# Gadersd/stable-diffusion-xl-burn

Hardware: AMD Instinct MI355X
Metric: images/sec SDXL-base 1024x1024 30-step CFG7.5 (whole job); UNet step ms p50 (higher is better)
Workload: dtype f16; 1 GPU; SDXL-base 1024x1024, n_steps=30 (31 CFG UNet step pairs), CFG 7.5, batch 1 prompt/GPU + VAE decode to u8 (BASELINE configs[1]); precision=f16, vae_dtype=f32_split, weights=synthetic seeded (random-init SDXL-base architecture), mix_classes=0, parallelism=replica x1, 1 prompt per GPU, weights broadcast once over RCCL, hipgraph=True, split_cfg=False, fused_xattn=True, pipelined_decode=False, prompts_per_call=1, full=False, library=stable-diffusion-xl-burn_amd/lib/libsdxl_mi355.so, debug_set=

## Files before the change

### stable-diffusion-xl-burn_amd/csrc/capi.hip

```cpp
#include "capi_internal.h"
#include <algorithm>
#include <cstring>

using namespace sdxl;

thread_local std::string sdxl::g_err;

namespace {
template <class H, class F> void create_handle(sdxl_ctx* ctx, H** out, F make) {
  std::unique_ptr<H> h(new H());
  h->ctx = ctx;
  make(*h);
  *out = h.release();
}
UNetCfg to_cfg(const sdxl_unet_config* c) {
  SDXL_REQUIRE(c != nullptr, "null config");
  SDXL_REQUIRE(c->n_levels >= 1 && c->n_levels <= 8, "n_levels out of range");
  UNetCfg u;
  u.adm_in_channels = c->adm_in_channels; u.in_channels = c->in_channels; u.out_channels = c->out_channels;
  u.model_channels = c->model_channels; u.n_head_channels = c->n_head_channels; u.context_dim = c->context_dim;
  u.is_refiner = c->is_refiner != 0;
  for (int i = 0; i < c->n_levels; ++i) { u.channel_mults.push_back(c->channel_mults[i]); u.transformer_depths.push_back(c->transformer_depths[i]); }
  SDXL_REQUIRE(u.model_channels > 0 && u.n_head_channels > 0 && u.context_dim > 0 && u.adm_in_channels > 0, "bad UNet config");
  return u;
// ... 72 lines not shown
  c->device = device_id;
  SDXL_HIP(hipStreamCreate(&c->stream));
  igemm_glds_init();
  attention_init();
  *out = c;
  API_END
}
int sdxl_debug_set(const char* key, int value) {
  API_BEGIN
  SDXL_REQUIRE(key != nullptr, "null key");
  if (std::strcmp(key, "igemm_variant") == 0) igemm_set_variant(value);
  else if (std::strcmp(key, "attn_variant") == 0) attention_set_variant(value);
  else if (std::strcmp(key, "igemm_epilogue_staged") == 0) igemm_set_epilogue_staged(value);
  else if (std::strcmp(key, "hl_weights_exact") == 0) igemm_set_hl_weights_exact(value);
  else if (std::strcmp(key, "igemm_wreg") == 0) igemm_set_wreg(value);
  else if (std::strcmp(key, "igemm_tsw") == 0) igemm_set_tsw(value);
  else if (std::strcmp(key, "igemm_warm") == 0) igemm_set_warm(value);
  else if (std::strcmp(key, "attn_xsplit") == 0) attention_set_xsplit(value);
  else if (std::strcmp(key, "splitk_wt") == 0) igemm_set_splitk_wt(value);
  else if (std::strcmp(key, "hl_demote") == 0) unet_set_hl_demote(value);
  else if (std::strcmp(key, "mix_classes") == 0) unet_set_mix_classes(value);
  else if (std::strcmp(key, "hl_tile96") == 0) igemm_set_hl_tile96(value);
  else if (std::strcmp(key, "wreg_xcd2d") == 0) igemm_set_wreg_xcd2d(value);
  else if (std::strcmp(key, "wide_db") == 0) igemm_set_wide_db(value);
#ifdef SDXL_MEASURE
  else if (std::strcmp(key, "igemm_unrolled") == 0) igemm_set_unrolled(value);
  else if (std::strcmp(key, "xa_vec64") == 0) igemm_set_xa_vec64(value);
  else if (std::strcmp(key, "no_cfg") == 0) g_debug_no_cfg = value != 0;
#endif
  else throw Error(std::string("unknown debug key ") + key);
// ... 539 lines not shown
```

### stable-diffusion-xl-burn_amd/csrc/capi_ops.hip

```cpp
#include "capi_internal.h"
#include <algorithm>
#include <cmath>

using namespace sdxl;

namespace {
__global__ void transpose_pad_kernel(const float* src, int lds_, int rows, int C, void* dst, int dt, int ldd) {
  const size_t i = (size_t)blockIdx.x * blockDim.x + threadIdx.x;
  if (i >= (size_t)rows * C) return;
  const int r = i / C, c = i - (size_t)r * C;
  const float v = src[(size_t)r * lds_ + c];
  if (dt == DT_F16) reinterpret_cast<_Float16*>(dst)[(size_t)c * ldd + r] = (_Float16)v;
  else reinterpret_cast<float*>(dst)[(size_t)c * ldd + r] = v;
}
__global__ void causal_mask_kernel(float* out, int n) {
  const int i = blockIdx.x * blockDim.x + threadIdx.x;
  if (i >= n * n) return;
  const int r = i / n, c = i - r * n;
  out[i] = c > r ? -INFINITY : 0.f;
}

struct Operand { std::string name; std::vector<int> shape; int kind; const float* data = nullptr; float eps = 0.f; int ld = 0; };
using Operands = std::vector<Operand>;
void add_linear(Operands& o, const std::string& n, int K, int N, const float* w, const float* b, int ld = 0) {
// ... 385 lines not shown
                                  const float* wq, const float* k, const float* v, int B, int Nq, int Nk, int C, int fused,
                                  float* out) {
  API_BEGIN
  SDXL_REQUIRE(ctx && x && gamma && beta && wq && k && v && out, "null argument");
  SDXL_REQUIRE(C % 64 == 0 && B >= 1 && Nq >= 1 && Nk >= 1, "State size must be a multiple of head size");
  use(ctx);
  hipStream_t s = pick(ctx, stream);
  const int M = B * Nq, vt_ld = (int)round_up(Nk, 64), H = C / 64;
  SDXL_REQUIRE(!fused || igemm_xattn_ok(DT_F16, DT_F16, M, C, C, Nq, Nk), "fused cross-attention: unsupported shape");
  Operands ops;
  add_linear(ops, "lin", C, C, wq, nullptr);
  add_norm(ops, "norm", C, gamma, beta, eps);
  Packed pk(ops, DT_F16, s);
  Tmp tmp;
  Exec ex; ex.s = s; ex.cdt = DT_F16; ex.sdt = DT_F16;
  const Lin l = pk.wb.linear_ln("lin", false, "norm");
  const F16Stream xs = identity_producer(ex, tmp, x, M, C, s);
  const Act xi(xs.rows, C, DT_F16);
  void* od = tmp.get((size_t)M * C * 2);
  Epi e; e.ln_stat = xs.stat; e.rpb = Nq;
  if (fused == 3) {
    float* q32 = (float*)tmp.get((size_t)M * C * 4);
    run_linear(ex, l, xi, M, Act(q32, C, DT_F32), e);
    void* khl = tmp.get((size_t)B * Nk * C * 4);
    void* vhl = tmp.get((size_t)B * C * vt_ld * 4);
    launch_f32_to_hl(k, C, khl, C, (size_t)B * Nk, C, s);
    launch_f32_to_hl(stage_vt(tmp, v, B, Nk, C, DT_F32, vt_ld, s), vt_ld, vhl, vt_ld, (size_t)B * C, vt_ld, s);
    AttnParams p = attn_params(q32, khl, vhl, vt_ld, od, C, DT_HL, B, H, Nq, Nk);
    p.q_dt = DT_F32; p.o_dt = DT_F16;
    SDXL_REQUIRE(launch_attention_d64_hl(p, s), "split-operand attention: unsupported shape");
  } else if (fused == 2) {
// ... 157 lines not shown
```

### stable-diffusion-xl-burn_amd/csrc/engine.h

```cpp
#pragma once
#include "kernels.h"

#include <map>
#include <memory>
#include <stdexcept>
#include <string>
#include <utility>
#include <vector>

namespace sdxl {

struct Error : std::runtime_error {
  explicit Error(const std::string& m) : std::runtime_error(m) {}
};
#define SDXL_HIP(x)                                                                                   \
  do {                                                                                                \
    hipError_t e__ = (x);                                                                             \
    if (e__ != hipSuccess) throw ::sdxl::Error(std::string(#x) + " failed: " + hipGetErrorString(e__)); \
  } while (0)
#define SDXL_REQUIRE(cond, msg)                          \
  do {                                                   \
    if (!(cond)) throw ::sdxl::Error(std::string(msg));  \
  } while (0)

// ... 96 lines not shown
  int dt;
  hipStream_t st;
  float* tmp = nullptr; size_t tmp_numel = 0;
  std::string last_fetched;
  WeightBuilder(const std::vector<ParamSpec>& sp, WeightSource& s, DeviceArena& a, int dtype, hipStream_t stream);
  ~WeightBuilder();
  bool wfrag = true;
  static size_t arena_bound(const std::vector<ParamSpec>& specs, int dt, bool wfrag = true);
  const ParamSpec& spec(const std::string& name, size_t* idx = nullptr) const;
  bool has(const std::string& name) const { return index.count(name) != 0; }
  const float* fetch(const std::string& name);
  Lin linear(const std::string& name, bool geglu = false, int dt_override = -1);
  Lin fused_linear(const std::vector<std::string>& names, int dt_override = -1);
  Lin linear_hilo(const std::string& name, bool geglu, bool dup = false, bool hl_interleave = false);
  float hl_scale(Lin& l, const std::vector<std::string>& weight_names);
  Lin linear_ln(const std::string& name, bool geglu, const std::string& norm);
  Lin fused_linear_ln(const std::vector<std::string>& names, const std::string& norm);
  Lin fold_ln(const std::vector<std::string>& names, const std::string& norm, bool geglu, int dt_override = -1, bool shadow = false, Lin* plain = nullptr, bool hilo_dup = false,
              bool hl_interleave = false);
  bool all_f16_exact(const std::vector<std::string>& names);
  float* tmp2 = nullptr; size_t tmp2_numel = 0;
  Lin conv(const std::string& name);
  void attach_wfrag(Lin& l, bool fill);
  NormW norm(const std::string& name);
};

struct Act {
  void* p = nullptr; int ld = 0; int dt = DT_F16;
  const float* gn_part = nullptr; int gn_rt = 0;
  const float* a_scale = nullptr;
  int a_scale_n = 1;
  Act() {}
  Act(void* p_, int ld_, int dt_) : p(p_), ld(ld_), dt(dt_) {}
  Act cols(int c0) const { Act a((char*)p + (size_t)c0 * dt_size(dt), ld, dt); a.a_scale = a_scale; a.a_scale_n = a_scale_n; return a; }
};

struct Profiler {
  enum { IGEMM = 0, ATTENTION = 1, GROUPNORM = 2, LAYERNORM = 3, OTHER = 4, NCLS = 5 };
// ... 322 lines not shown
```

### stable-diffusion-xl-burn_amd/csrc/igemm_common.h

```cpp
#pragma once
#include "kernels.h"
#include <stdexcept>
#include <type_traits>

namespace sdxl {

typedef _Float16 half_t;
typedef _Float16 half8 __attribute__((ext_vector_type(8)));
typedef _Float16 half4 __attribute__((ext_vector_type(4)));
typedef float f32x4 __attribute__((ext_vector_type(4)));
typedef float f32x16 __attribute__((ext_vector_type(16)));

typedef const __attribute__((address_space(1))) void* gptr_t;
typedef float f32x8 __attribute__((ext_vector_type(8)));
__device__ __forceinline__ f32x8 uniform_load8(const float* ptr) {
  const unsigned long long a = (unsigned long long)(uintptr_t)ptr;
  const unsigned long long u = ((unsigned long long)__builtin_amdgcn_readfirstlane((unsigned)(a >> 32)) << 32) | (unsigned)__builtin_amdgcn_readfirstlane((unsigned)a);
  return *(const __attribute__((address_space(4))) f32x8*)(uintptr_t)u;
}
__device__ __forceinline__ f32x4 col_vec4(const float* arr, bool present, int nbu, int fh, const void* zeros) {
  const f32x8 c = uniform_load8(present ? arr + nbu : reinterpret_cast<const float*>(zeros));
  return fh ? f32x4{c[4], c[5], c[6], c[7]} : f32x4{c[0], c[1], c[2], c[3]};
}
typedef __attribute__((address_space(3))) void* lptr_t;
// ... 888 lines not shown
    const float inv = 1.0f / l;
#pragma unroll
    for (int dt = 0; dt < 2; ++dt) {
      f32x16 o;
#pragma unroll
      for (int r = 0; r < 16; ++r) o[r] = 0.f;
#pragma unroll
      for (int s6 = 0; s6 < 6; ++s6) o = __builtin_amdgcn_mfma_f32_32x32x16_f16(vf[dt][s6], pf[s6], o, 0, 0, 0);
#pragma unroll
      for (int r = 0; r < 16; ++r) acc[i][dt][r] = o[r] * inv;
    }
    lnA[i] = 1.f; lnC[i] = 0.f;
  }
}

template <int TM>
__device__ __forceinline__ void xattn_inplace_hl(const IgemmParams& p, f32x16 (&acc)[TM][2], int mw, int nw, int lane,
                                                 float (&lnA)[TM], float (&lnC)[TM], const void* zeros) {
  static_assert(TM == 1, "split-precision fused cross-attention: one-MFMA-row wave tiles");
  if (nw >= p.N) return;
  const int fh = lane >> 5;
  const int nctx = p.xa_nctx;
  const int mclamp = mw < p.M ? mw : p.M - 1;
  const int b = __builtin_amdgcn_readfirstlane(mclamp / p.rpb);
  const size_t foff = ((size_t)b * (p.N >> 6) + (nw >> 6)) * (24 * 64) + lane;
  const half8* fhi = reinterpret_cast<const half8*>(p.xa_k) + foff;
  const half8* flo = reinterpret_cast<const half8*>(p.xa_k_lo) + foff;
  half8 kh[3][4], kl[3][4];
#pragma unroll
  for (int t = 0; t < 3; ++t)
// ... 94 lines not shown
```

### stable-diffusion-xl-burn_amd/csrc/igemm_glds.hip

```cpp
#include "igemm_common.h"
#include <atomic>

namespace sdxl {

template <int BM, int BN, int NS, int MINB = 2>
__global__ __launch_bounds__(256, MINB) void igemm_glds_kernel(const IgemmParams p, const void* zeros) {
  kernarg_prefetch<(int)sizeof(IgemmParams) + 8>();
  constexpr int WM = BM / 2, WN = BN / 2;
  constexpr int TM = WM / 32, TN = WN / 32;
  constexpr int AJ = BM / 32, BJ = BN / 32;
  constexpr int PER = AJ + BJ;
  constexpr int KT = 64;
  constexpr int STAGE = (BM + BN) * 128;
  extern __shared__ __attribute__((aligned(16))) char smem[];

  const int tid = threadIdx.x, lane = tid & 63;
  const int wave = __builtin_amdgcn_readfirstlane(tid >> 6);
  const int wm = wave >> 1, wn = wave & 1;

  const int tilesN = (p.N + BN - 1) / BN;
  const int nwg = gridDim.x;
  int bid = blockIdx.x;
  {
    const int q = nwg >> 3, r = nwg & 7, xcd = bid & 7, idx = bid >> 3;
// ... 994 lines not shown
      const int g = f - 12, d = 32 * (g / 6) + fr, key = 16 * (g % 6) + sub;
      if (key < nctx) x = Vt[((size_t)b * C + h * 64 + d) * vt_ld + key];
    }
    v[e] = x;
  }
  out[i] = v;
}
size_t xattn_pack_bytes(int B, int C) { return (size_t)B * (C / 64) * 24 * 64 * 16; }
void launch_xattn_pack(const void* K, const void* Vt, void* out, int B, int C, int nctx, int vt_ld, hipStream_t s) {
  const size_t n = (size_t)B * (C / 64) * 24 * 64;
  hipLaunchKernelGGL(xattn_pack_kernel, dim3((unsigned)((n + 255) / 256)), dim3(256), 0, s, reinterpret_cast<const half_t*>(K),
                     reinterpret_cast<const half_t*>(Vt), reinterpret_cast<half8*>(out), B, C, nctx, vt_ld);
}

bool launch_igemm_wreg(const IgemmParams& p, int variant, hipStream_t s);
bool launch_igemm_glds(const IgemmParams& p, int variant, hipStream_t s) {
  if (!g_zero_pages[current_device()]) return false;
  if (p.act > 1) return false;
  if (p.a_dt != DT_F16 || (p.Cin % 64) != 0 || (p.lda % 8) != 0 || (p.Kpad % 64) != 0) return false;
  if ((reinterpret_cast<uintptr_t>(p.A) & 15) != 0) return false;
  if (p.n_split < p.N && (p.n_split & 3) != 0) return false;
  if (p.ebias && (p.ebias_ld & 3) != 0) return false;
  if (p.stat_out && (variant == 2 || variant == 5 || variant == 19 || variant == 38)) return false;
  const bool was_auto = variant == 0;
  IgemmParams psk = p;
  psk.splitk = 1;
  psk.splitk_wt = g_splitk_wt.load();
  if (p.xa_k) {
    if (p.act != 0 || p.n_split < p.N || p.stat_out || p.R || p.ebias ||
        !igemm_xattn_ok(p.a_dt, p.c_dt, p.M, p.N, p.K, p.rpb, p.xa_nctx))
      throw std::runtime_error("igemm: fused cross-attention needs a plain f16 projection (no residual / split outputs)");
    if (!p.xa_k_lo && p.c_dt != DT_F16) throw std::runtime_error("igemm: the f16 fused cross-attention writes f16 rows");
    const int nk = p.Kpad / 64;
    if (p.xa_k_lo) {
      const double c128 = tile_cost(p.M, p.N, nk, 128, 128, 1.0), c96 = tile_cost(p.M, p.N, nk, 96, 128, 1.0);
      if (c96 < c128) launch_pipe<96, 128, 3, 3, 6, half_t, true, false, false, true>(psk, s);
      else launch_pipe<128, 128, 4, 4, 8, half_t, true, false, false, true>(psk, s);
      return true;
    }
    int v = variant;
    if (v != 35 && v != 36 && v != 44 && v != 45) {
      const double c256 = tile_cost(p.M, p.N, nk, 256, 128, 1.0), c128 = tile_cost(p.M, p.N, nk, 128, 128, 1.0), c96 = tile_cost(p.M, p.N, nk, 96, 128, 1.0);
      v = c256 <= c128 && c256 <= c96 ? 35 : (c96 < c128 ? 45 : (nk >= 40 ? 44 : 36));
    }
    if (v == 35) launch_pipe<256, 128, 3, 4, 8, half_t, true>(psk, s);
    else if (v == 36) launch_pipe<128, 128, 4, 4, 8, half_t, true>(psk, s);
    else if (v == 44) launch_pipe<128, 128, 5, 4, 8, half_t, true>(psk, s);
    else launch_pipe<96, 128, 3, 3, 6, half_t, true>(psk, s);
    return true;
  }
  if (p.gn_part) {
    if (!igemm_gn_part_ok(p)) throw std::runtime_error("igemm: GroupNorm statistics requested from a shape the 256x128 epilogue does not take");
    variant = 0;
  }
  if (p.shadow) {
// ... 116 lines not shown
```

### stable-diffusion-xl-burn_amd/csrc/igemm_wreg.hip

```cpp
#include "igemm_common.h"
#include <atomic>

namespace sdxl {

template <int OFF> __device__ __forceinline__ half8 wreg_gload128(const half_t* ptr) {
  half8 v;
  asm volatile("global_load_dwordx4 %0, %1, off offset:%2" : "=v"(v) : "v"(ptr), "n"(OFF));
  return v;
}

__global__ void repack_wfrag_kernel(const f32x4* __restrict__ src, f32x4* __restrict__ dst, int nblocks, int nk) {
  const size_t i = (size_t)blockIdx.x * blockDim.x + threadIdx.x;
  const size_t total = (size_t)nblocks * nk * 256;
  if (i >= total) return;
  const int lane = (int)(i & 63), kk = (int)((i >> 6) & 3);
  const size_t t = i >> 8;
  const int kt = (int)(t % nk);
  const int nb = (int)(t / nk);
  dst[i] = src[(size_t)(nb * 32 + (lane & 31)) * (nk * 8) + kt * 8 + kk * 2 + (lane >> 5)];
}
void launch_repack_wfrag(const void* w, void* wf, int Npad, int Kpad, hipStream_t s) {
  const int nblocks = Npad / 32, nk = Kpad / 64;
  const size_t total = (size_t)nblocks * nk * 256;
  hipLaunchKernelGGL(repack_wfrag_kernel, dim3((unsigned)((total + 255) / 256)), dim3(256), 0, s, reinterpret_cast<const f32x4*>(w),
// ... 137 lines not shown
  if (part == 0 && fh == 0) {
#pragma unroll
    for (int i = 0; i < TM; ++i) {
      const int r2 = (i * 32 + fr) * 2;
      const float s1 = (A1[i] + xsum[r2]) + (xsum[TM * 64 + r2] + xsum[2 * TM * 64 + r2]);
      const float s2 = (A2[i] + xsum[r2 + 1]) + (xsum[TM * 64 + r2 + 1] + xsum[2 * TM * 64 + r2 + 1]);
      if (mok[i]) {
        float* dst = p.stat_out + ((size_t)(nw >> 6) * p.M + m[i]) * 2;
        dst[0] = piv[i] + s1 * (1.0f / 64.0f);
        dst[1] = fmaxf(s2 - s1 * s1 * (1.0f / 64.0f), 0.f);
      }
    }
  }
}

#ifdef SDXL_MEASURE
__device__ unsigned* g_wreg_tl = nullptr;
void igemm_set_wreg_timeline(void* buf) {
  unsigned* b = reinterpret_cast<unsigned*>(buf);
  if (hipMemcpyToSymbol(HIP_SYMBOL(g_wreg_tl), &b, sizeof(b)) != hipSuccess) throw std::runtime_error("igemm_wreg: cannot set the timeline buffer");
}
#define WREG_STAMP(i) do { wtl[i] = (unsigned)__builtin_amdgcn_s_memtime(); } while (0)
#else
#define WREG_STAMP(i) do { } while (0)
#endif
constexpr int wreg_mode_flags(int m) {
  return m >= 16 ? m : m == 1 ? 16 : m == 2 ? 32 : m == 3 ? 64 : m == 4 ? 128 : m == 5 ? 256 : m == 6 ? 512 : m == 7 ? 1024 : m == 8 ? 2048 : 0;
}
template <int BM, int L, int MODE = 0>
__global__ __launch_bounds__(512) void igemm_wreg_kernel(const IgemmParams p, const void* zeros) {
#ifdef SDXL_MEASURE
  unsigned wtl[8] = {0, 0, 0, 0, 0, 0, 0, 0};
  wtl[6] = (unsigned)__builtin_amdgcn_s_memrealtime();
#endif
  WREG_STAMP(0);
  kernarg_prefetch<(int)sizeof(IgemmParams) + 8>();
  constexpr int NG = 2;
  constexpr int NSG = L + 1;
  constexpr int TM = BM / 32;
  constexpr int PP = BM / 32;
  constexpr int FL = wreg_mode_flags(MODE);
  constexpr bool NOMFMA = FL & 16, FROZEN = FL & 32, NOVMEM = FL & 64, NOBAR = FL & 128, XCDALT = FL & 256, NOA = FL & 512, NOWL = FL & 1024,
                 ACONTIG = FL & 2048, NOLDS = FL & 4096;
  constexpr int NW = NOWL ? 0 : 4;
// ... 184 lines not shown
    for (int pass = (ns - first) / NSG; pass > 0; --pass) {
      static_for<L>([&](auto C) { ktile(std::integral_constant<int, decltype(C)::value + 1>{}, STEADY{}); });
      ktile(I0{}, STEADY{});
    }
  }
  static_for<L>([&](auto X) {
    constexpr int D = L - decltype(X)::value;
    if (D <= nkg) ktile(std::integral_constant<int, L + 1 - D>{}, std::integral_constant<int, D>{});
  });
  WREG_STAMP(3);
  if constexpr (!NOBAR) { if ((nk & 1) && g == 1) __builtin_amdgcn_s_barrier(); }
  asm volatile("" ::: "memory");
  __builtin_amdgcn_sched_barrier(0);

  WregEpiOperands<TM> eop;
  wreg_epilogue_request<TM>(p, m0, n0 + w * 32, lane, g, zeros, eop);
  static_assert(4 * TM * 2 * 64 * 16 <= L * SLOT, "a group's four exchange pieces must fit its dead slots 0 .. L - 1");
  f32x4* xw = reinterpret_cast<f32x4*>(smem + g * RING) + (size_t)w * (TM * 2 * 64) + lane;
  const f32x4* xo = reinterpret_cast<const f32x4*>(smem + (1 - g) * RING) + (size_t)w * (TM * 2 * 64) + lane;
#pragma unroll
  for (int i = 0; i < TM; ++i)
#pragma unroll
    for (int qq = 0; qq < 2; ++qq) {
      f32x4 v;
#pragma unroll
      for (int r = 0; r < 4; ++r) v[r] = g ? acc[i][4 * qq + r] : acc[i][8 + 4 * qq + r];
      xw[(i * 2 + qq) * 64] = v;
    }
  wait_lgkmcnt<0>();
  __builtin_amdgcn_s_barrier();
  asm volatile("" ::: "memory");
#pragma unroll
  for (int i = 0; i < TM; ++i)
#pragma unroll
    for (int qq = 0; qq < 2; ++qq) {
      const f32x4 o = xo[(i * 2 + qq) * 64];
#pragma unroll
      for (int r = 0; r < 4; ++r) {
        if (g) acc[i][8 + 4 * qq + r] = o[r] + acc[i][8 + 4 * qq + r];
        else acc[i][4 * qq + r] = acc[i][4 * qq + r] + o[r];
      }
    }
  WREG_STAMP(4);
  static_assert((2 * BM + 6 * 2 * BM) * 4 <= SLOT, "statistics exchange must fit one slot");
  float* xch = reinterpret_cast<float*>(smem + L * SLOT);
  wreg_epilogue<TM>(p, acc, m0, n0 + w * 32, lane, w, g, xch, eop);
#ifdef SDXL_MEASURE
  WREG_STAMP(5);
  asm volatile("s_waitcnt vmcnt(0)" ::: "memory");
  wtl[7] = (unsigned)__builtin_amdgcn_s_memrealtime();
  { const unsigned t6 = (unsigned)__builtin_amdgcn_s_memtime();
    if (g_wreg_tl && lane == 0) { unsigned* d = g_wreg_tl + ((size_t)blockIdx.x * 8 + wave) * 16; for (int i = 0; i < 8; ++i) d[i] = wtl[i]; d[8] = t6; } }
#endif
}

static std::atomic<int> g_wreg_enable{1};
void igemm_set_wreg(int v) { g_wreg_enable = v; }
static std::atomic<int> g_wreg_xcd2d{0};
void igemm_set_wreg_xcd2d(int v) { g_wreg_xcd2d = v; }

static int wreg_warm_groups(const IgemmParams& p, int ntiles) {
  if (!p.warm[0] || !p.warm_bytes[0] || ntiles > 512) return 0;
  const int spare = (ntiles <= 256 ? 256 : 512) - ntiles;
  return spare < 8 ? 0 : spare > 64 ? 64 : spare;
}
template <int BM, int L, int MODE = 0>
static void launch_wreg_t(const IgemmParams& p, hipStream_t s) {
  constexpr size_t lds = (size_t)2 * (L + 1) * BM * 128;
  static_assert(lds >= (size_t)8 * (BM / 32) * 2048 + (size_t)(2 * BM + 6 * 2 * BM) * 4, "exchange areas must fit the dead rings");
  static bool attr_set[kIgemmMaxDev] = {};
  const int dev = igemm_current_device();
  if (!attr_set[dev]) {
    if (hipFuncSetAttribute(reinterpret_cast<const void*>(&igemm_wreg_kernel<BM, L, MODE>), hipFuncAttributeMaxDynamicSharedMemorySize, (int)lds) != hipSuccess)
      throw std::runtime_error("igemm_wreg: hipFuncSetAttribute(MaxDynamicSharedMemorySize) failed");
    attr_set[dev] = true;
  }
  const int tilesM = (p.M + BM - 1) / BM, tilesN = p.N / 128;
  const int ntiles = tilesM * tilesN;
  IgemmParams q = p;
  q.wreg_xcd2d = g_wreg_xcd2d.load();
  hipLaunchKernelGGL((igemm_wreg_kernel<BM, L, MODE>), dim3(ntiles + wreg_warm_groups(p, ntiles)), dim3(512), lds, s, q, igemm_zero_page());
}

bool igemm_wreg_ok(const IgemmParams& p) {
  if (!p.Wf || !igemm_zero_page()) return false;
  if (p.a_dt != DT_F16 || (p.c_dt != DT_F16 && p.c_dt != DT_F32)) return false;
  if (p.ksize != 1 || p.stride != 1 || p.up != 0 || p.pad != 0 || p.Hin != p.Hout || p.Win != p.Wout) return false;
  if (p.N % 128 != 0 || p.Cin != p.K || p.K != p.Kpad || p.Kpad % 64 != 0 || p.Kpad < 128) return false;
  if (p.act != 0 || p.n_split < p.N || p.xa_k || p.gn_part || p.ln_stat || p.acc_scale) return false;
  if ((p.lda & 7) != 0 || (reinterpret_cast<uintptr_t>(p.A) & 15) != 0) return false;
  if ((p.ldc & 7) != 0 || (reinterpret_cast<uintptr_t>(p.C) & 15) != 0) return false;
  if (p.R && ((p.ldr & 7) != 0 || (reinterpret_cast<uintptr_t>(p.R) & 15) != 0)) return false;
  if (p.ebias) return false;
  if (p.shadow && (p.c_dt != DT_F32 || !p.shadow_gamma || (p.shadow_ld & (p.shadow_lo_scale < 0.f ? 15 : 7)) != 0 || (reinterpret_cast<uintptr_t>(p.shadow) & 15) != 0)) return false;
  return true;
}
// ... 29 lines not shown
  if (variant == 74) { launch_wreg_t<96, 2, 16 | 32 | 4096>(p, s); return true; }
  if (variant == 75) { launch_wreg_t<96, 2, 16 | 32 | 4096 | 128>(p, s); return true; }
  if (variant == 76) { launch_wreg_t<96, 2, 16 | 4096>(p, s); return true; }
  if (variant == 77) { launch_wreg_t<96, 2, 4096>(p, s); return true; }
#endif
  int bm = variant == 60 ? 96 : variant == 62 ? 64 : 0;
  if (!bm) {
    const long t64 = (long)((p.M + 63) / 64) * (p.N / 128);
    bm = t64 <= 256 ? 64 : 96;
  }
  if (bm == 64) launch_wreg_t<64, 2>(p, s);
  else launch_wreg_t<96, 2>(p, s);
  return true;
}

}
```

### stable-diffusion-xl-burn_amd/csrc/kernels.h

```cpp
#pragma once
#include <hip/hip_runtime.h>
#include <stdint.h>

namespace sdxl {

enum DType : int { DT_F32 = 0, DT_F16 = 1, DT_HL = 2 };

static inline size_t dt_size(int dt) { return dt == DT_F16 ? 2 : 4; }

struct IgemmParams {
  const void* A;
  const void* W;
  const void* Wf;
  int a_dt;
  int B, Hin, Win, Cin, lda;
  int Hout, Wout;
  int ksize, stride, pad, up;
  int M, N, K, Kpad;
  const float* bias;
  const float* ebias;
  int ebias_ld;
  int rpb;
  int act;
  const void* R; int ldr; int r_dt;
// ... 19 lines not shown
  void* shadow; int shadow_ld; const float* shadow_gamma;
  float shadow_lo_scale;
};
bool igemm_gn_part_ok(const IgemmParams& p);
bool igemm_xattn_ok(int a_dt, int c_dt, int M, int N, int K, int rpb, int n_ctx);
size_t xattn_pack_bytes(int B, int C);
void launch_xattn_pack(const void* K, const void* Vt, void* out, int B, int C, int n_ctx, int vt_ld, hipStream_t s);
int igemm_splitk_slices(const IgemmParams& p);
size_t igemm_splitk_ws_bytes(int batch, int rows_per_entry, int n_max);
constexpr int kSplitkCounters = 4096;
void launch_igemm(const IgemmParams& p, int compute_dt, hipStream_t s);
void launch_repack_wfrag(const void* w, void* wf, int Npad, int Kpad, hipStream_t s);
bool igemm_wreg_ok(const IgemmParams& p);
void igemm_set_tsw(int v);
bool igemm_wreg_selected(const IgemmParams& p);
void igemm_set_warm(int v);
int igemm_warm_enabled();
void igemm_set_splitk_wt(int v);
void igemm_set_hl_tile96(int v);
void igemm_set_wreg_xcd2d(int v);
void igemm_set_wide_db(int v);
void igemm_set_wreg(int v);
void igemm_set_variant(int v);
void igemm_set_hl_weights_exact(int v);
void igemm_set_xa_vec64(int v);
void igemm_set_epilogue_staged(int v);
void igemm_set_unrolled(int v);
#ifdef SDXL_MEASURE
void igemm_set_timeline(void* device_buf);
void igemm_set_wreg_timeline(void* device_buf);
// ... 147 lines not shown
```

### stable-diffusion-xl-burn_amd/csrc/unet.cpp

```cpp
#include "engine.h"

#include <atomic>
#include <cmath>
#include <cstring>

namespace sdxl {

namespace {
ResBlockW load_res(WeightBuilder& wb, const std::string& p, int cin, int cout, std::vector<std::string>& emb_names,
                   int& emb_off) {
  ResBlockW r;
  r.cin = cin; r.cout = cout;
  r.norm_in = wb.norm(p + ".norm_in");
  r.conv_in = wb.conv(p + ".conv_in");
  r.norm_out = wb.norm(p + ".norm_out");
  r.conv_out = wb.conv(p + ".conv_out");
  r.has_skip = wb.has(p + ".skip_connection.weight");
  if (r.has_skip) r.skip = wb.conv(p + ".skip_connection");
  r.emb_off = emb_off;
  emb_names.push_back(p + ".lin_embed");
  emb_off += cout;
  return r;
}
const std::vector<std::string> kQkv = {".attn1.query", ".attn1.key", ".attn1.value"};
// ... 49 lines not shown
  }
}
namespace {
STW load_st(WeightBuilder& wb, const std::string& p, int C, int heads, int depth, bool fuse_ln, const StPlan& plan) {
  STW s;
  s.C = C; s.heads = heads; s.plan = plan;
  s.norm = wb.norm(p + ".norm");
  s.proj_in = wb.linear(p + ".proj_in");
  for (int j = 0; j < depth; ++j) {
    const std::string q = p + ".blocks." + std::to_string(j);
    const std::vector<std::string> qkv = {q + kQkv[0], q + kQkv[1], q + kQkv[2]};
    TBlockW t;
    if (fuse_ln) {
      t.qkv = wb.fused_linear_ln(qkv, q + ".norm1");
      t.out1 = wb.linear(q + kOut1);
      t.q2 = wb.linear_ln(q + kQ2, false, q + ".norm2");
      t.kv2 = wb.fused_linear({q + ".attn2.key", q + ".attn2.value"});
      t.out2 = wb.linear(q + kOut2);
      t.geglu = wb.linear_ln(q + kGeglu, true, q + ".norm3");
      t.ff = wb.linear(q + kFf);
      s.blocks.push_back(t);
      continue;
    }
    t.n1 = wb.norm(q + ".norm1");
    t.qkv = pack_proj(wb, plan.qkv, qkv, false, plan.qkv_sh ? &t.qkv_sh : nullptr, q + ".norm1");
    t.out1 = pack_proj(wb, plan.out1, {q + kOut1}, false);
    t.n2 = wb.norm(q + ".norm2");
    t.q2 = pack_proj(wb, plan.q2, {q + kQ2}, false, plan.q2_sh ? &t.q2_sh : nullptr, q + ".norm2");
    t.kv2 = wb.fused_linear({q + ".attn2.key", q + ".attn2.value"});
    t.out2 = pack_proj(wb, plan.out2, {q + kOut2}, false);
    t.n3 = wb.norm(q + ".norm3");
// ... 785 lines not shown
```

### stable-diffusion-xl-burn_amd/csrc/weights.cpp

```cpp
#include "engine.h"

#include <cstdio>
#include <cstdlib>
#include <cstring>
#include <cmath>

namespace sdxl {

DeviceArena::~DeviceArena() { if (base) (void)hipFree(base); }
void DeviceArena::reserve(size_t bytes) {
  if (bytes <= cap && base) return;
  if (base) { SDXL_HIP(hipFree(base)); base = nullptr; }
  SDXL_HIP(hipMalloc((void**)&base, bytes));
  cap = bytes;
}
void* DeviceArena::alloc(size_t bytes) {
  const size_t a = round_up(off, 256);
  off = a + bytes;
  if (off > peak) peak = off;
  if (dry) return (void*)(uintptr_t)(a + 256);
  if (off > cap) throw Error("device arena overflow (" + std::to_string(off) + " > " + std::to_string(cap) + ")");
  return base + a;
}

// ... 112 lines not shown
  for (const std::string& n : weight_names) launch_absmax(fetch(n), spec(n).numel(), sc, st, true);
  float h = 0.f;
  SDXL_HIP(hipMemcpyAsync(&h, sc, sizeof(float), hipMemcpyDeviceToHost, st));
  SDXL_HIP(hipStreamSynchronize(st));
  int e = 0;
  if (h > 0.f && std::isfinite(h)) { (void)std::frexp(h, &e); e = 14 - e; }
  e = e > 24 ? 24 : (e < -24 ? -24 : e);
  const float wscale = std::ldexp(1.0f, e), inv = 1.0f / wscale;
  SDXL_HIP(hipMemcpyAsync(sc, &inv, sizeof(float), hipMemcpyHostToDevice, st));
  SDXL_HIP(hipStreamSynchronize(st));
  bool first = true;
  for (const std::string& n : weight_names) { launch_f16_exact(fetch(n), spec(n).numel(), wscale, sc + 1, st, !first); first = false; }
  return wscale;
}

void WeightBuilder::attach_wfrag(Lin& l, bool fill) {
  const int wdt = l.dt >= 0 ? l.dt : dt;
  if (!wfrag) return;
  if (wdt != DT_F16 || l.ksize != 1 || l.N % 128 != 0 || l.K != l.Kpad || l.Kpad % 64 != 0 || l.Kpad < 128 || l.cs || l.acc_scale) return;
  void* wf = arena.alloc((size_t)l.Npad * l.Kpad * 2);
  l.wf = wf;
  if (fill) launch_repack_wfrag(l.w, wf, l.Npad, l.Kpad, st);
}
Lin WeightBuilder::linear(const std::string& name, bool geglu, int dt_override) {
  const ParamSpec& s = spec(name + ".weight");
  Lin l; l.K = s.shape[0]; l.N = s.shape[1]; l.ksize = 1; l.cin = l.K;
  const int wdt = dt_override >= 0 ? dt_override : ((dt == DT_HL && l.K % 32 != 0) ? DT_F32 : dt);
  if (wdt != dt) l.dt = wdt;
  const int kt = wdt == DT_F16 ? 64 : 32;
  l.Kpad = (int)round_up(l.K, kt); l.Npad = (int)round_up(l.N, 128);
  void* w = arena.alloc((size_t)l.Npad * l.Kpad * dt_size(wdt));
  float* b = (float*)arena.alloc((size_t)l.Npad * sizeof(float));
  l.w = w; l.b = b;
  const float wscale = wdt == DT_HL ? hl_scale(l, {name + ".weight"}) : 1.f;
// ... 46 lines not shown
  if (src.empty()) return l;
  SDXL_HIP(hipMemsetAsync(w, 0, (size_t)l.Npad * l.Kpad * dt_size(wdt), st));
  SDXL_HIP(hipMemsetAsync(b, 0, (size_t)l.Npad * sizeof(float), st));
  int off = 0;
  for (const std::string& n : names) {
    const ParamSpec& s = spec(n + ".weight");
    const int N = s.shape[1];
    launch_pack_linear(fetch(n + ".weight"), w, wdt, l.K, N, l.Kpad, N, 0, off, st, nullptr, wscale);
    const float* bsrc = has(n + ".bias") ? fetch(n + ".bias") : nullptr;
    launch_pack_bias(bsrc, b, N, N, 0, off, st);
    off += N;
  }
  l.w = w; l.b = b;
  return l;
}
Lin WeightBuilder::linear_ln(const std::string& name, bool geglu, const std::string& norm) {
  return fold_ln({name}, norm, geglu);
}
Lin WeightBuilder::fused_linear_ln(const std::vector<std::string>& names, const std::string& norm) {
  return fold_ln(names, norm, false);
}
bool WeightBuilder::all_f16_exact(const std::vector<std::string>& names) {
  if (src.empty() || names.empty()) return true;
  float* flag = (float*)tmp2;
  if (tmp2_numel < 4) { if (tmp2) SDXL_HIP(hipFree(tmp2)); SDXL_HIP(hipMalloc((void**)&tmp2, 64 * sizeof(float))); tmp2_numel = 64; flag = tmp2; }
  bool first = true;
  for (const std::string& n : names) { launch_f16_exact(fetch(n), spec(n).numel(), 1.0f, flag, st, !first); first = false; }
  float h = 0.f;
  SDXL_HIP(hipMemcpyAsync(&h, flag, sizeof(float), hipMemcpyDeviceToHost, st));
  SDXL_HIP(hipStreamSynchronize(st));
  return h != 0.f;
}
// ... 155 lines not shown
  if (e.shadow) {
    p.shadow = e.shadow; p.shadow_ld = e.shadow_ld; p.shadow_gamma = e.shadow_gamma; p.shadow_lo_scale = e.shadow_lo_scale;
    const bool ok = (w.dt >= 0 ? w.dt : ex.cdt) == DT_F16 && igemm_wreg_selected(p);
    if (!ok) { p.shadow = nullptr; p.shadow_gamma = nullptr; p.stat_out = nullptr; p.shadow_lo_scale = 0.f; }
    if (e.shadow_done) *e.shadow_done = ok;
  }
  SDXL_REQUIRE(!e.xa_k || igemm_xattn_ok(a.dt, out.dt, p.M, p.N, p.K, p.rpb, e.xa_nctx), "fused cross-attention: unsupported shape");
  SDXL_REQUIRE(!e.ln_stat || (w.ln_k ? w.ln_k : w.K) % 64 == 0, "LayerNorm-folded GEMM needs K % 64 == 0");
  SDXL_REQUIRE(!e.stat_out || (w.N % 64 == 0 && (e.n_split < 0 || e.n_split >= w.N) && e.act == 0), "row statistics need a plain N % 64 == 0 output");
  SDXL_REQUIRE(!e.ln_stat || w.cs, "ln_stat given but the weight is not LayerNorm-folded");
  SDXL_REQUIRE(!w.cs || e.ln_stat, "LayerNorm-folded weight used without row statistics");
  SDXL_REQUIRE(!((w.dt >= 0 ? w.dt : ex.cdt) == DT_F32 && a.dt != DT_F32), "f32 compute needs f32 activations");
  if (ex.prof) ex.prof->begin(Profiler::IGEMM, 2.0 * p.M * (double)p.N * p.K, ex.s, p.M, p.N, p.K, p.ksize, e.cls);
  if (ex.warm && (w.dt >= 0 ? w.dt : ex.cdt) == DT_F16) {
    WarmSeq& ws = *ex.warm;
    const bool host = igemm_wreg_selected(p);
    const size_t wbytes = (size_t)w.Npad * w.Kpad * 2;
    const char* lo; const char* hi;
    if (host) {
      const char* f = reinterpret_cast<const char*>(p.Wf), *b = reinterpret_cast<const char*>(w.b);
      lo = (b && b < f && f - b <= (64 << 10)) ? b : f;
      hi = f + wbytes;
    } else {
      lo = reinterpret_cast<const char*>(p.W); hi = lo + wbytes;
      auto ext = [&](const void* q, size_t sz) { const char* c = reinterpret_cast<const char*>(q); if (q && c >= hi && c - hi <= (64 << 10)) hi = c + sz; };
      ext(w.b, (size_t)w.Npad * 4); ext(w.cs, (size_t)w.Npad * 4); ext(w.ln_eps, 4);
    }
    if (ws.recording) {
      if (p.xa_k) ws.seq.push_back(WarmSeq::Item{p.xa_k, (unsigned)xattn_pack_bytes(p.M / p.rpb, p.N), false, 0u, {nullptr, nullptr, nullptr}, {0u, 0u, 0u}});
      const unsigned budget = host ? 14u << 20 : 0u;
      ws.seq.push_back(WarmSeq::Item{lo, (unsigned)(hi - lo), host, budget, {nullptr, nullptr, nullptr}, {0u, 0u, 0u}});
// ... 88 lines not shown
```

Baseline: 1.423 images/sec.

## Fuse cross-attention into weight-register GEMM epilogue for LN-folded query projection

Adds an XA variant of the weight-register (wreg) GEMM kernel. Its epilogue applies the LayerNorm fold and bias to the query projection, stages q fragments in LDS, and runs a short cross-attention unit per wave (at most 96 context tokens) with MFMA, writing the attention output directly. LN-folded query weights now get repacked weight fragments so this path qualifies, and the warm-up scheduler treats it as a host-warmed GEMM. The aim is to remove the separate query write/read and the attention launch for attn2. In exchange it adds register pressure and a specialised kernel with many eligibility conditions.

```diff
diff --git a/stable-diffusion-xl-burn_amd/csrc/capi.hip b/stable-diffusion-xl-burn_amd/csrc/capi.hip
--- a/stable-diffusion-xl-burn_amd/csrc/capi.hip
+++ b/stable-diffusion-xl-burn_amd/csrc/capi.hip
@@ -110,6 +110,7 @@
   else if (std::strcmp(key, "igemm_epilogue_staged") == 0) igemm_set_epilogue_staged(value);
   else if (std::strcmp(key, "hl_weights_exact") == 0) igemm_set_hl_weights_exact(value);
   else if (std::strcmp(key, "igemm_wreg") == 0) igemm_set_wreg(value);
+  else if (std::strcmp(key, "wreg_xattn") == 0) igemm_set_wreg_xattn(value);
   else if (std::strcmp(key, "igemm_tsw") == 0) igemm_set_tsw(value);
   else if (std::strcmp(key, "igemm_warm") == 0) igemm_set_warm(value);
   else if (std::strcmp(key, "attn_xsplit") == 0) attention_set_xsplit(value);
diff --git a/stable-diffusion-xl-burn_amd/csrc/capi_ops.hip b/stable-diffusion-xl-burn_amd/csrc/capi_ops.hip
--- a/stable-diffusion-xl-burn_amd/csrc/capi_ops.hip
+++ b/stable-diffusion-xl-burn_amd/csrc/capi_ops.hip
@@ -423,7 +423,7 @@
   Packed pk(ops, DT_F16, s);
   Tmp tmp;
   Exec ex; ex.s = s; ex.cdt = DT_F16; ex.sdt = DT_F16;
-  const Lin l = pk.wb.linear_ln("lin", false, "norm");
+  const Lin l = pk.wb.linear_ln("lin", false, "norm", true);
   const F16Stream xs = identity_producer(ex, tmp, x, M, C, s);
   const Act xi(xs.rows, C, DT_F16);
   void* od = tmp.get((size_t)M * C * 2);
diff --git a/stable-diffusion-xl-burn_amd/csrc/engine.h b/stable-diffusion-xl-burn_amd/csrc/engine.h
--- a/stable-diffusion-xl-burn_amd/csrc/engine.h
+++ b/stable-diffusion-xl-burn_amd/csrc/engine.h
@@ -134,14 +134,14 @@
   Lin fused_linear(const std::vector<std::string>& names, int dt_override = -1);
   Lin linear_hilo(const std::string& name, bool geglu, bool dup = false, bool hl_interleave = false);
   float hl_scale(Lin& l, const std::vector<std::string>& weight_names);
-  Lin linear_ln(const std::string& name, bool geglu, const std::string& norm);
+  Lin linear_ln(const std::string& name, bool geglu, const std::string& norm, bool xattn_query = false);
   Lin fused_linear_ln(const std::vector<std::string>& names, const std::string& norm);
   Lin fold_ln(const std::vector<std::string>& names, const std::string& norm, bool geglu, int dt_override = -1, bool shadow = false, Lin* plain = nullptr, bool hilo_dup = false,
               bool hl_interleave = false);
   bool all_f16_exact(const std::vector<std::string>& names);
   float* tmp2 = nullptr; size_t tmp2_numel = 0;
   Lin conv(const std::string& name);
-  void attach_wfrag(Lin& l, bool fill);
+  void attach_wfrag(Lin& l, bool fill, bool folded = false);
   NormW norm(const std::string& name);
 };
 
diff --git a/stable-diffusion-xl-burn_amd/csrc/igemm_common.h b/stable-diffusion-xl-burn_amd/csrc/igemm_common.h
--- a/stable-diffusion-xl-burn_amd/csrc/igemm_common.h
+++ b/stable-diffusion-xl-burn_amd/csrc/igemm_common.h
@@ -926,6 +926,51 @@
   }
 }
 
+__device__ __forceinline__ void xattn_unit(const half8 (&qf)[4], const half8 (&kf)[3][4], const half8 (&vf)[2][6], int nctx, int fh, f32x16 (&o)[2]) {
+  f32x16 sv[3];
+#pragma unroll
+  for (int t = 0; t < 3; ++t) {
+#pragma unroll
+    for (int r = 0; r < 16; ++r) sv[t][r] = 0.f;
+#pragma unroll
+    for (int s4 = 0; s4 < 4; ++s4) sv[t] = __builtin_amdgcn_mfma_f32_32x32x16_f16(kf[t][s4], qf[s4], sv[t], 0, 0, 0);
+  }
+  float mx = -INFINITY;
+#pragma unroll
+  for (int t = 0; t < 3; ++t)
+#pragma unroll
+    for (int r = 0; r < 16; ++r) {
+      if (32 * t + 8 * (r >> 2) + 4 * fh + (r & 3) >= nctx) sv[t][r] = -INFINITY;
+      mx = fmaxf(mx, sv[t][r]);
+    }
+  mx = fmaxf(mx, __shfl_xor(mx, 32));
+  float l = 0.f;
+  half8 pf[6];
+#pragma unroll
+  for (int s6 = 0; s6 < 6; ++s6) {
+    float ls = 0.f;
+#pragma unroll
+    for (int e = 0; e < 8; ++e) {
+      const float pe = __builtin_amdgcn_exp2f(sv[s6 >> 1][8 * (s6 & 1) + e] - mx);
+      ls += pe;
+      pf[s6][e] = (half_t)pe;
+    }
+    l += ls;
+  }
+  l += __shfl_xor(l, 32);
+  const float inv = 1.0f / l;
+#pragma unroll
+  for (int dt = 0; dt < 2; ++dt) {
+    f32x16 a;
+#pragma unroll
+    for (int r = 0; r < 16; ++r) a[r] = 0.f;
+#pragma unroll
+    for (int s6 = 0; s6 < 6; ++s6) a = __builtin_amdgcn_mfma_f32_32x32x16_f16(vf[dt][s6], pf[s6], a, 0, 0, 0);
+#pragma unroll
+    for (int r = 0; r < 16; ++r) o[dt][r] = a[r] * inv;
+  }
+}
+
 template <int TM>
 __device__ __forceinline__ void xattn_inplace_hl(const IgemmParams& p, f32x16 (&acc)[TM][2], int mw, int nw, int lane,
                                                  float (&lnA)[TM], float (&lnC)[TM], const void* zeros) {
diff --git a/stable-diffusion-xl-burn_amd/csrc/igemm_glds.hip b/stable-diffusion-xl-burn_amd/csrc/igemm_glds.hip
--- a/stable-diffusion-xl-burn_amd/csrc/igemm_glds.hip
+++ b/stable-diffusion-xl-burn_amd/csrc/igemm_glds.hip
@@ -1032,6 +1032,7 @@
 }
 
 bool launch_igemm_wreg(const IgemmParams& p, int variant, hipStream_t s);
+bool launch_igemm_wreg_xattn(const IgemmParams& p, int variant, hipStream_t s);
 bool launch_igemm_glds(const IgemmParams& p, int variant, hipStream_t s) {
   if (!g_zero_pages[current_device()]) return false;
   if (p.act > 1) return false;
@@ -1057,6 +1058,7 @@
       return true;
     }
     int v = variant;
+    if (v != 35 && v != 36 && v != 44 && v != 45 && launch_igemm_wreg_xattn(psk, v, s)) return true;
     if (v != 35 && v != 36 && v != 44 && v != 45) {
       const double c256 = tile_cost(p.M, p.N, nk, 256, 128, 1.0), c128 = tile_cost(p.M, p.N, nk, 128, 128, 1.0), c96 = tile_cost(p.M, p.N, nk, 96, 128, 1.0);
       v = c256 <= c128 && c256 <= c96 ? 35 : (c96 < c128 ? 45 : (nk >= 40 ? 44 : 36));
diff --git a/stable-diffusion-xl-burn_amd/csrc/igemm_wreg.hip b/stable-diffusion-xl-burn_amd/csrc/igemm_wreg.hip
--- a/stable-diffusion-xl-burn_amd/csrc/igemm_wreg.hip
+++ b/stable-diffusion-xl-burn_amd/csrc/igemm_wreg.hip
@@ -175,6 +175,97 @@
   }
 }
 
+template <int BM> struct WregXaOperands {
+  LnCoop<BM, 4 * BM> ln;
+  half8 kf[3][4], vf[2][6];
+  f32x4 cz[2], bz[2];
+  bool unit;
+};
+template <int BM>
+__device__ __forceinline__ void wreg_xattn_request(const IgemmParams& p, int m0, int n0, int lane, int wave, const void* zeros, WregXaOperands<BM>& op) {
+  constexpr int TM = BM / 32;
+  static_assert((4 * BM) % 64 == 0 && 4 * BM <= 512 && LnCoop<BM, 4 * BM>::OK, "four statistics threads per tile row, whole waves");
+  const int g = wave >> 2, w = wave & 3, fh = lane >> 5;
+  if (wave < 4 * BM / 64) op.ln.load(p, m0, wave * 64 + lane);
+  const int mu = m0 + 32 * (wave >> 1);
+  op.unit = wave < 2 * TM && mu < p.M;
+  if (op.unit) {
+    const int b = __builtin_amdgcn_readfirstlane(mu / p.rpb);
+    const half8* fx = reinterpret_cast<const half8*>(p.xa_k) + ((size_t)b * (p.N >> 6) + ((n0 >> 6) + (wave & 1))) * (24 * 64) + lane;
+#pragma unroll
+    for (int t = 0; t < 3; ++t)
+#pragma unroll
+      for (int s4 = 0; s4 < 4; ++s4) op.kf[t][s4] = fx[(t * 4 + s4) * 64];
+#pragma unroll
+    for (int dt = 0; dt < 2; ++dt)
+#pragma unroll
+      for (int s6 = 0; s6 < 6; ++s6) op.vf[dt][s6] = fx[(12 + dt * 6 + s6) * 64];
+  }
+  const int nb = n0 + 32 * w + 16 * g;
+#pragma unroll
+  for (int q = 0; q < 2; ++q) {
+    op.cz[q] = col_vec4(p.ln_cs, p.ln_stat != nullptr, nb + 8 * q, fh, zeros);
+    op.bz[q] = col_vec4(p.bias, p.bias != nullptr, nb + 8 * q, fh, zeros);
+  }
+}
+template <int BM>
+__device__ __forceinline__ void wreg_xattn_coef(const IgemmParams& p, int m0, int lane, int wave, WregXaOperands<BM>& op, float* coef) {
+  const int tid = wave * 64 + lane;
+  if (p.ln_stat != nullptr && p.ln_slots <= 24) {
+    if (wave < 4 * BM / 64) op.ln.finish(p, m0, coef);
+  } else if (tid < BM) {
+    float a, c;
+    ln_row_coef(p, m0 + tid, a, c);
+    coef[tid * 2] = a; coef[tid * 2 + 1] = c;
+  }
+}
+template <int BM, int L>
+__device__ __forceinline__ void wreg_xattn_tail(const IgemmParams& p, const f32x16 (&acc)[BM / 32], int m0, int n0, int lane, int wave, char* smem,
+                                                const float* coef, const WregXaOperands<BM>& op) {
+  constexpr int TM = BM / 32, SLOT = BM * 128, RING = (L + 1) * SLOT;
+  static_assert(TM * 4 * 1024 == SLOT, "a head's q fragments fill one ring slot");
+  const int fr = lane & 31, fh = lane >> 5, g = wave >> 2, w = wave & 3;
+  const float sc = p.xa_scale * 1.44269504088896340736f;
+  half8* qx = reinterpret_cast<half8*>(smem + (w >> 1) * RING + L * SLOT) + (2 * (w & 1) + g) * 64 + lane;
+#pragma unroll
+  for (int i = 0; i < TM; ++i) {
+    const float lna = coef[(i * 32 + fr) * 2], lnc = coef[(i * 32 + fr) * 2 + 1];
+    half8 qf;
+#pragma unroll
+    for (int e = 0; e < 8; ++e) {
+      const float a = g ? acc[i][8 + e] : acc[i][e];
+      qf[e] = (half_t)((lna * a + lnc * op.cz[e >> 2][e & 3] + op.bz[e >> 2][e & 3]) * sc);
+    }
+    qx[i * 256] = qf;
+  }
+  wait_lgkmcnt<0>();
+  __builtin_amdgcn_s_barrier();
+  asm volatile("" ::: "memory");
+  if (!op.unit) return;
+  const int ui = wave >> 1, uh = wave & 1;
+  const half8* qr = reinterpret_cast<const half8*>(smem + uh * RING + L * SLOT) + ui * 256 + lane;
+  half8 qf[4];
+#pragma unroll
+  for (int s4 = 0; s4 < 4; ++s4) qf[s4] = qr[s4 * 64];
+  f32x16 o[2];
+  xattn_unit(qf, op.kf, op.vf, p.xa_nctx, fh, o);
+  const int m = m0 + 32 * ui + fr;
+  half_t* crow = reinterpret_cast<half_t*>(p.C) + (size_t)(m < p.M ? m : 0) * p.ldc + n0 + 64 * uh + 8 * fh;
+#pragma unroll
+  for (int dt = 0; dt < 2; ++dt)
+#pragma unroll
+    for (int t = 0; t < 2; ++t) {
+      half8 h;
+#pragma unroll
+      for (int r = 0; r < 4; ++r) {
+        const auto sw = __builtin_amdgcn_permlane32_swap(__float_as_uint(o[dt][8 * t + r]), __float_as_uint(o[dt][8 * t + 4 + r]), false, false);
+        h[r] = (half_t)__uint_as_float(sw[0]);
+        h[4 + r] = (half_t)__uint_as_float(sw[1]);
+      }
+      if (m < p.M) *reinterpret_cast<half8*>(crow + 32 * dt + 16 * t) = h;
+    }
+}
+
 #ifdef SDXL_MEASURE
 __device__ unsigned* g_wreg_tl = nullptr;
 void igemm_set_wreg_timeline(void* buf) {
@@ -188,7 +279,7 @@
 constexpr int wreg_mode_flags(int m) {
   return m >= 16 ? m : m == 1 ? 16 : m == 2 ? 32 : m == 3 ? 64 : m == 4 ? 128 : m == 5 ? 256 : m == 6 ? 512 : m == 7 ? 1024 : m == 8 ? 2048 : 0;
 }
-template <int BM, int L, int MODE = 0>
+template <int BM, int L, int MODE = 0, bool XA = false>
 __global__ __launch_bounds__(512) void igemm_wreg_kernel(const IgemmParams p, const void* zeros) {
 #ifdef SDXL_MEASURE
   unsigned wtl[8] = {0, 0, 0, 0, 0, 0, 0, 0};
@@ -403,7 +494,10 @@
   __builtin_amdgcn_sched_barrier(0);
 
   WregEpiOperands<TM> eop;
-  wreg_epilogue_request<TM>(p, m0, n0 + w * 32, lane, g, zeros, eop);
+  WregXaOperands<XA ? BM : 64> xop;
+  float* const xa_coef = reinterpret_cast<float*>(smem + NG * RING);
+  if constexpr (XA) { static_assert(MODE == 0, "production arithmetic only"); wreg_xattn_request<BM>(p, m0, n0, lane, wave, zeros, xop); }
+  else wreg_epilogue_request<TM>(p, m0, n0 + w * 32, lane, g, zeros, eop);
   static_assert(4 * TM * 2 * 64 * 16 <= L * SLOT, "a group's four exchange pieces must fit its dead slots 0 .. L - 1");
   f32x4* xw = reinterpret_cast<f32x4*>(smem + g * RING) + (size_t)w * (TM * 2 * 64) + lane;
   const f32x4* xo = reinterpret_cast<const f32x4*>(smem + (1 - g) * RING) + (size_t)w * (TM * 2 * 64) + lane;
@@ -416,6 +510,7 @@
       for (int r = 0; r < 4; ++r) v[r] = g ? acc[i][4 * qq + r] : acc[i][8 + 4 * qq + r];
       xw[(i * 2 + qq) * 64] = v;
     }
+  if constexpr (XA) wreg_xattn_coef<BM>(p, m0, lane, wave, xop, xa_coef);
   wait_lgkmcnt<0>();
   __builtin_amdgcn_s_barrier();
   asm volatile("" ::: "memory");
@@ -433,7 +528,8 @@
   WREG_STAMP(4);
   static_assert((2 * BM + 6 * 2 * BM) * 4 <= SLOT, "statistics exchange must fit one slot");
   float* xch = reinterpret_cast<float*>(smem + L * SLOT);
-  wreg_epilogue<TM>(p, acc, m0, n0 + w * 32, lane, w, g, xch, eop);
+  if constexpr (XA) wreg_xattn_tail<BM, L>(p, acc, m0, n0, lane, wave, smem, xa_coef, xop);
+  else wreg_epilogue<TM>(p, acc, m0, n0 + w * 32, lane, w, g, xch, eop);
 #ifdef SDXL_MEASURE
   WREG_STAMP(5);
   asm volatile("s_waitcnt vmcnt(0)" ::: "memory");
@@ -453,14 +549,14 @@
   const int spare = (ntiles <= 256 ? 256 : 512) - ntiles;
   return spare < 8 ? 0 : spare > 64 ? 64 : spare;
 }
-template <int BM, int L, int MODE = 0>
+template <int BM, int L, int MODE = 0, bool XA = false>
 static void launch_wreg_t(const IgemmParams& p, hipStream_t s) {
-  constexpr size_t lds = (size_t)2 * (L + 1) * BM * 128;
+  constexpr size_t lds = (size_t)2 * (L + 1) * BM * 128 + (XA ? BM * 8 : 0);
   static_assert(lds >= (size_t)8 * (BM / 32) * 2048 + (size_t)(2 * BM + 6 * 2 * BM) * 4, "exchange areas must fit the dead rings");
   static bool attr_set[kIgemmMaxDev] = {};
   const int dev = igemm_current_device();
   if (!attr_set[dev]) {
-    if (hipFuncSetAttribute(reinterpret_cast<const void*>(&igemm_wreg_kernel<BM, L, MODE>), hipFuncAttributeMaxDynamicSharedMemorySize, (int)lds) != hipSuccess)
+    if (hipFuncSetAttribute(reinterpret_cast<const void*>(&igemm_wreg_kernel<BM, L, MODE, XA>), hipFuncAttributeMaxDynamicSharedMemorySize, (int)lds) != hipSuccess)
       throw std::runtime_error("igemm_wreg: hipFuncSetAttribute(MaxDynamicSharedMemorySize) failed");
     attr_set[dev] = true;
   }
@@ -468,7 +564,7 @@
   const int ntiles = tilesM * tilesN;
   IgemmParams q = p;
   q.wreg_xcd2d = g_wreg_xcd2d.load();
-  hipLaunchKernelGGL((igemm_wreg_kernel<BM, L, MODE>), dim3(ntiles + wreg_warm_groups(p, ntiles)), dim3(512), lds, s, q, igemm_zero_page());
+  hipLaunchKernelGGL((igemm_wreg_kernel<BM, L, MODE, XA>), dim3(ntiles + wreg_warm_groups(p, ntiles)), dim3(512), lds, s, q, igemm_zero_page());
 }
 
 bool igemm_wreg_ok(const IgemmParams& p) {
@@ -528,4 +624,34 @@
   return true;
 }
 
-}
+static std::atomic<int> g_wreg_xattn{1};
+void igemm_set_wreg_xattn(int v) { g_wreg_xattn = v; }
+static bool wreg_xattn_ok(const IgemmParams& p) {
+  if (!p.xa_k || p.xa_k_lo || !p.Wf || !igemm_zero_page()) return false;
+  if (p.a_dt != DT_F16 || p.c_dt != DT_F16) return false;
+  if (p.ksize != 1 || p.stride != 1 || p.up != 0 || p.pad != 0 || p.Hin != p.Hout || p.Win != p.Wout) return false;
+  if (p.N % 128 != 0 || p.Cin != p.K || p.K != p.Kpad || p.Kpad % 64 != 0 || p.Kpad < 128) return false;
+  if (p.act != 0 || p.n_split < p.N || p.gn_part || p.acc_scale || p.stat_out || p.R || p.ebias || p.shadow) return false;
+  if (p.rpb <= 0 || p.rpb % 64 != 0 || p.M % p.rpb != 0 || p.xa_nctx < 1 || p.xa_nctx > 96) return false;
+  if ((p.lda & 7) != 0 || (reinterpret_cast<uintptr_t>(p.A) & 15) != 0) return false;
+  if ((p.ldc & 7) != 0 || (reinterpret_cast<uintptr_t>(p.C) & 15) != 0) return false;
+  return true;
+}
+bool igemm_wreg_xattn_selected(const IgemmParams& p) {
+  if (!wreg_xattn_ok(p) || !g_wreg_enable.load() || !g_wreg_xattn.load()) return false;
+  const long rows = 2L * p.rpb;
+  return ((rows + 95) / 96) * (long)(p.N / 128) <= 512;
+}
+bool launch_igemm_wreg_xattn(const IgemmParams& p, int variant, hipStream_t s) {
+  if (!igemm_wreg_xattn_selected(p)) return false;
+  int bm = variant == 60 ? 96 : variant == 62 ? 64 : 0;
+  if (!bm) {
+    const long t64 = (long)((p.M + 63) / 64) * (p.N / 128);
+    bm = t64 <= 256 ? 64 : 96;
+  }
+  if (bm == 64) launch_wreg_t<64, 2, 0, true>(p, s);
+  else launch_wreg_t<96, 2, 0, true>(p, s);
+  return true;
+}
+
+}
diff --git a/stable-diffusion-xl-burn_amd/csrc/kernels.h b/stable-diffusion-xl-burn_amd/csrc/kernels.h
--- a/stable-diffusion-xl-burn_amd/csrc/kernels.h
+++ b/stable-diffusion-xl-burn_amd/csrc/kernels.h
@@ -57,6 +57,8 @@
 bool igemm_wreg_ok(const IgemmParams& p);
 void igemm_set_tsw(int v);
 bool igemm_wreg_selected(const IgemmParams& p);
+bool igemm_wreg_xattn_selected(const IgemmParams& p);
+void igemm_set_wreg_xattn(int v);
 void igemm_set_warm(int v);
 int igemm_warm_enabled();
 void igemm_set_splitk_wt(int v);
diff --git a/stable-diffusion-xl-burn_amd/csrc/unet.cpp b/stable-diffusion-xl-burn_amd/csrc/unet.cpp
--- a/stable-diffusion-xl-burn_amd/csrc/unet.cpp
+++ b/stable-diffusion-xl-burn_amd/csrc/unet.cpp
@@ -87,7 +87,7 @@
     if (fuse_ln) {
       t.qkv = wb.fused_linear_ln(qkv, q + ".norm1");
       t.out1 = wb.linear(q + kOut1);
-      t.q2 = wb.linear_ln(q + kQ2, false, q + ".norm2");
+      t.q2 = wb.linear_ln(q + kQ2, false, q + ".norm2", true);
       t.kv2 = wb.fused_linear({q + ".attn2.key", q + ".attn2.value"});
       t.out2 = wb.linear(q + kOut2);
       t.geglu = wb.linear_ln(q + kGeglu, true, q + ".norm3");
diff --git a/stable-diffusion-xl-burn_amd/csrc/weights.cpp b/stable-diffusion-xl-burn_amd/csrc/weights.cpp
--- a/stable-diffusion-xl-burn_amd/csrc/weights.cpp
+++ b/stable-diffusion-xl-burn_amd/csrc/weights.cpp
@@ -150,10 +150,10 @@
   return wscale;
 }
 
-void WeightBuilder::attach_wfrag(Lin& l, bool fill) {
+void WeightBuilder::attach_wfrag(Lin& l, bool fill, bool folded) {
   const int wdt = l.dt >= 0 ? l.dt : dt;
   if (!wfrag) return;
-  if (wdt != DT_F16 || l.ksize != 1 || l.N % 128 != 0 || l.K != l.Kpad || l.Kpad % 64 != 0 || l.Kpad < 128 || l.cs || l.acc_scale) return;
+  if (wdt != DT_F16 || l.ksize != 1 || l.N % 128 != 0 || l.K != l.Kpad || l.Kpad % 64 != 0 || l.Kpad < 128 || (l.cs && !folded) || l.acc_scale) return;
   void* wf = arena.alloc((size_t)l.Npad * l.Kpad * 2);
   l.wf = wf;
   if (fill) launch_repack_wfrag(l.w, wf, l.Npad, l.Kpad, st);
@@ -230,8 +230,10 @@
   l.w = w; l.b = b;
   return l;
 }
-Lin WeightBuilder::linear_ln(const std::string& name, bool geglu, const std::string& norm) {
-  return fold_ln({name}, norm, geglu);
+Lin WeightBuilder::linear_ln(const std::string& name, bool geglu, const std::string& norm, bool xattn_query) {
+  Lin l = fold_ln({name}, norm, geglu);
+  if (xattn_query && !geglu && !l.k_form) attach_wfrag(l, !src.empty(), true);
+  return l;
 }
 Lin WeightBuilder::fused_linear_ln(const std::vector<std::string>& names, const std::string& norm) {
   return fold_ln(names, norm, false);
@@ -417,7 +419,7 @@
   if (ex.prof) ex.prof->begin(Profiler::IGEMM, 2.0 * p.M * (double)p.N * p.K, ex.s, p.M, p.N, p.K, p.ksize, e.cls);
   if (ex.warm && (w.dt >= 0 ? w.dt : ex.cdt) == DT_F16) {
     WarmSeq& ws = *ex.warm;
-    const bool host = igemm_wreg_selected(p);
+    const bool host = igemm_wreg_selected(p) || igemm_wreg_xattn_selected(p);
     const size_t wbytes = (size_t)w.Npad * w.Kpad * 2;
     const char* lo; const char* hi;
     if (host) {
```

Measured after the change: 1.442 images/sec (median of 6 runs). 1.3% higher.
